# amolrpatil21/PorQua

Hardware: AMD Instinct MI355X
Metric: QPs solved/sec (rebalance dates) at N=1000 assets, 1-8 GPU; x vs host CPU (higher is better)
Workload: dtype f64; 1 GPU; config3: long-only min-variance (P=2*Pearson cov, budget + box [0,1]), daily rebalance; n_assets=1000, window=252, dates_per_gpu=4749, global_batch=4749, parallelism=dates-sharded x1

## Files before the change

include/porqua_hip.h:

```cpp
#ifndef PORQUA_HIP_H
#define PORQUA_HIP_H

#include <stdint.h>

#ifdef __cplusplus
extern "C" {
#endif

#define PQ_VERSION 100

#define PQ_UNSOLVED 0
#define PQ_SOLVED 1
#define PQ_SOLVED_INACCURATE 2
#define PQ_MAX_ITER 3
#define PQ_NEED_REFACTOR 4
#define PQ_PRIMAL_INFEASIBLE (-3)
#define PQ_DUAL_INFEASIBLE (-4)
#define PQ_NON_CONVEX (-5)

#define PQ_OUT_OBJ 0
#define PQ_OUT_PRIM 1
#define PQ_OUT_DUAL 2
#define PQ_OUT_GAP 3
#define PQ_OUT_RHO 4
// ... 155 lines not shown
  double* grho;
  double* M; double* Minv; int32_t k_ld; int64_t M_stride;
  double* aq; int64_t aq_stride;
  double* hinv; int32_t ldh;
  int32_t gmax;
} pq_gcap;
int pq_gcap_assemble(const pq_lowrank* lr, const pq_problem* pb, const pq_gcap* gc, const pq_settings* s,
                     const double* band, int64_t ldo, int32_t r0, const double* pc, int64_t ldpc,
                     const double* cc, void* stream);
int pq_gcap_prepare(const pq_lowrank* lr, const pq_problem* pb, pq_state* st, const pq_gcap* gc,
                    const pq_settings* s, const int32_t* idx, int32_t nidx, const double* band, int64_t ldo,
                    int32_t r0, const double* pc, int64_t ldpc, void* stream);
int pq_admm_lr_gcap(const pq_lowrank* lr, const pq_problem* pb, pq_state* st, const pq_gcap* gc,
                    const pq_settings* s, int32_t iters_this_call, const double* pc, int64_t ldpc, int32_t r0,
                    const double* cc, const int32_t* cg_nzr, const double* cg_nzv, int32_t nzmax, void* stream);
int pq_gcap_form(int32_t gmax, int32_t mg);

int pq_eigcap_form(const pq_lowrank* lr, const pq_problem* pb, const pq_state* st, const pq_settings* s,
                   const int32_t* pdate, const double* V, const double* evals, const double* What,
                   const double* cc, int32_t k_ld, const int32_t* idx, int32_t nidx, double* Minv,
                   int64_t M_stride, double* scratch, void* stream);

int pq_polish_batched(const pq_problem* pb, pq_state* st, const int32_t* idx, int32_t nidx,
                      const pq_settings* s, void* stream);

int pq_polish_lr_batched(const pq_lowrank* lr, const pq_problem* pb, pq_state* st,
                         const int32_t* idx, int32_t nidx, const pq_settings* s, void* stream);

int pq_polish_w_batched(const pq_lowrank* lr, const pq_problem* pb, pq_state* st, const int32_t* idx,
                        int32_t nidx, const pq_settings* s, int32_t ldk, int32_t final_try,
                        const double* band, int64_t ldo, int32_t r0, void* stream);

#define PQ_PG_RECORD 384
#define PQ_PG_PASS_SCRATCH 123537
#define PQ_PG_PENDING 0
#define PQ_PG_DONE 1
#define PQ_PG_FALLBACK 2
#define PQ_PG_SKIP 3
#define PQ_PG_WMB 8
#define PQ_PG_WSCR(k_ld) (2 * PQ_PG_WMB * (int64_t)(k_ld))
typedef struct pq_pg_wide {
  const pq_gcap* gc;
  const double* pc; int64_t ldpc; int32_t r0; const double* cc;
  const int32_t* nzr; const double* nzv; int32_t nzmax;
  double* wscr; int64_t wscr_stride;
  int32_t refine_steps;
} pq_pg_wide;
int pq_polish_grouped_init(const pq_lowrank* lr, const pq_problem* pb, pq_state* st, double* rec,
                           const pq_settings* s, void* stream);
int pq_polish_grouped_round(const pq_lowrank* lr, const pq_problem* pb, pq_state* st, double* rec, int32_t ldk,
                            const int32_t* gdates, int32_t ngroups, const int32_t* urows, const int32_t* ucnt,
                            const int32_t* uoff, int32_t umax, const pq_settings* s, double* pass_scratch,
                            const pq_pg_wide* wide, void* stream);

int pq_simulate_periods(const double* panel, int64_t ldp, int32_t n, const double* W, int64_t ldw,
                        const int32_t* row0, const int32_t* nrows, int32_t nper,
                        const int64_t* ret_off, const int32_t* ret_day, double fc,
                        double days_per_year, double* ret, double* wend, int64_t ldwe,
                        double* turnover, int32_t rescale, void* stream);

int pq_gemv_batched(const double* U, int64_t ldu, int64_t su, int32_t m, int32_t n, int32_t batch,
                    int32_t trans, const double* x, int64_t sx, double* y, int64_t sy, void* stream);

int pq_lad_mv_batched(const double* M, int64_t ldm, int64_t sm, int32_t n, int32_t batch,
                      const double* V, int64_t sv, int32_t k, const double* S, int64_t ss,
                      double* out, int64_t so, void* stream);

int pq_wgram_batched(const double* U, int64_t ldu, int64_t su, int32_t k, int32_t n, int32_t batch,
                     const double* w, int64_t sw, const double* r, int64_t sr, const double* d, int64_t sd,
                     double* M, int32_t k_ld, int64_t sm, void* stream);

int64_t pq_workspace_bytes(int32_t n, int32_t batch, int32_t mg, int32_t path, int32_t tmax, int32_t ldk);


int64_t pq_sym_eig_work_doubles(int32_t ld);
int pq_sym_eig_batched(double* A, int32_t ld, int64_t a_stride, int32_t n, int32_t batch, double* V,
                       int64_t v_stride, double* evals, int64_t e_stride, double* work, int64_t w_stride,
                       int32_t max_sweeps, double tol, void* stream);

int pq_sym_eig_converged(const double* work, int32_t ld, int64_t w_stride, int32_t batch, int32_t max_sweeps,
                         int32_t* conv, void* stream);

int pq_psd_form_batched(const double* V, int64_t v_stride, const double* evals, int64_t e_stride, int32_t ld,
                        int32_t n, int32_t batch, double* out, int64_t o_stride, void* stream);

int pq_tile_gemm_batched(const double* A, int64_t sa, int32_t ta, const double* B, int64_t sb, int32_t tb,
                         double* C, int64_t sc, int32_t ld, int32_t batch, void* stream);

#define PQ_PCT_OK 0
#define PQ_PCT_EMPTY_BUCKET 1
#define PQ_PCT_NAN_SCORE 2
#define PQ_PCT_MAX_N 16384
#define PQ_PCT_MAX_BUCKETS 256
int pq_percentile_batched(const double* scores, int64_t lds, int32_t n, int32_t batch, double sign,
                          int32_t n_percentiles, const int32_t* prev, const int32_t* next,
                          const double* gamma, double* th, int32_t* bucket, int32_t* counts, double* w,
                          int32_t* status, void* stream);

int pq_shrink_stats_band(const double* band, int64_t ldo, int32_t r0, int32_t nrows, int32_t W,
                         const int32_t* rows, int64_t ld_rows, const int32_t* tlen, int32_t tmax,
                         int32_t batch, int32_t n, int32_t centred, int32_t kind, double* stats,
                         void* stream);

#define PQ_RP_OK 0
#define PQ_RP_MAX_SWEEPS 1
#define PQ_RP_BAD_INPUT 2
// ... 63 lines not shown
```

porqua_amd/_lib.py:

```python
from __future__ import annotations

import ctypes
import os

_HERE = os.path.dirname(os.path.abspath(__file__))
LIB_PATH = os.environ.get("PQ_LIB_PATH") or os.path.join(_HERE, "libporqua_hip.so")

c_int32 = ctypes.c_int32
c_int64 = ctypes.c_int64
c_dp = ctypes.c_void_p

PQ_UNSOLVED = 0
PQ_SOLVED = 1
PQ_SOLVED_INACCURATE = 2
PQ_MAX_ITER = 3
PQ_NEED_REFACTOR = 4
PQ_PRIMAL_INFEASIBLE = -3
PQ_DUAL_INFEASIBLE = -4
PQ_NON_CONVEX = -5

PQ_PCT_OK, PQ_PCT_EMPTY_BUCKET, PQ_PCT_NAN_SCORE = range(3)
PQ_PCT_MAX_N = 16384
PQ_PCT_MAX_BUCKETS = 256

# ... 143 lines not shown
    "pq_init_state_lr": ([ctypes.POINTER(PQLowRank), ctypes.POINTER(PQProblem), ctypes.POINTER(PQState), c_dp,
                          c_int32, ctypes.POINTER(PQSettings), c_dp], c_int32),
    "pq_polish_w_batched": ([ctypes.POINTER(PQLowRank), ctypes.POINTER(PQProblem), ctypes.POINTER(PQState),
                             c_dp, c_int32, ctypes.POINTER(PQSettings), c_int32, c_int32, c_dp, c_int64,
                             c_int32, c_dp], c_int32),
    "pq_gram_xy_grouped": ([c_dp, c_int64, c_int32, c_dp, c_dp, c_int32, c_dp, c_int32, c_dp, c_dp, c_dp,
                            c_int64, c_dp, c_dp, c_int64, c_dp], c_int32),
    "pq_gram_xy_batched": ([c_dp, c_int64, c_int32, c_dp, c_dp, c_dp, c_int32, c_int32, c_dp, c_int64,
                            c_dp, c_dp], c_int32),
    "pq_init_state": ([ctypes.POINTER(PQProblem), ctypes.POINTER(PQState), c_dp, c_int32,
                       ctypes.POINTER(PQSettings), c_dp], c_int32),
    "pq_factor_batched": ([ctypes.POINTER(PQProblem), ctypes.POINTER(PQState), c_dp, c_int32,
                           ctypes.POINTER(PQSettings), c_int32, c_dp], c_int32),
    "pq_factor_last_route": ([], c_int32),
    "pq_factor_res_prof": ([c_dp, c_int32], c_int32),
    "pq_factor_large": ([ctypes.POINTER(PQProblem), ctypes.POINTER(PQState), c_dp, c_int32,
                         ctypes.POINTER(PQSettings), c_int32, c_dp, c_int64, c_dp], c_int32),
    "pq_sym_eig_work_doubles": ([c_int32], c_int64),
    "pq_sym_eig_batched": ([c_dp, c_int32, c_int64, c_int32, c_int32, c_dp, c_int64, c_dp, c_int64, c_dp, c_int64,
                            c_int32, ctypes.c_double, c_dp], c_int32),
    "pq_sym_eig_converged": ([c_dp, c_int32, c_int64, c_int32, c_int32, c_dp, c_dp], c_int32),
    "pq_psd_form_batched": ([c_dp, c_int64, c_dp, c_int64, c_int32, c_int32, c_int32, c_dp, c_int64, c_dp], c_int32),
    "pq_tile_gemm_batched": ([c_dp, c_int64, c_int32, c_dp, c_int64, c_int32, c_dp, c_int64, c_int32, c_int32,
                              c_dp], c_int32),
    "pq_admm_batched": ([ctypes.POINTER(PQProblem), ctypes.POINTER(PQState), c_dp, c_int32,
                         ctypes.POINTER(PQSettings), c_int32, c_dp], c_int32),
    "pq_polish_batched": ([ctypes.POINTER(PQProblem), ctypes.POINTER(PQState), c_dp, c_int32,
                           ctypes.POINTER(PQSettings), c_dp], c_int32),
    "pq_admm_lr_grouped": ([ctypes.POINTER(PQLowRank), ctypes.POINTER(PQProblem), ctypes.POINTER(PQState),
                            c_dp, c_int32, c_int64, c_dp, c_int32, c_dp, c_dp, c_dp, c_int32,
                            ctypes.POINTER(PQSettings), c_int32, c_dp, c_int64, c_int32, c_dp, c_dp, c_dp,
                            c_int32, c_dp], c_int32),
    "pq_admm_lr_sweep": ([ctypes.POINTER(PQLowRank), ctypes.POINTER(PQProblem), ctypes.POINTER(PQState),
                          c_dp, c_int32, c_int64, c_dp, c_int32, ctypes.POINTER(PQSettings), c_int32, c_dp,
                          c_int64, c_int32, c_dp, c_int32, c_dp, c_int64, c_dp], c_int32),
    "pq_sweep_scratch_doubles": ([c_int32, c_int32, c_int32], c_int64),
    "pq_polish_lr_batched": ([ctypes.POINTER(PQLowRank), ctypes.POINTER(PQProblem), ctypes.POINTER(PQState),
                              c_dp, c_int32, ctypes.POINTER(PQSettings), c_dp], c_int32),
    "pq_lr_capacitance": ([ctypes.POINTER(PQLowRank), ctypes.POINTER(PQProblem), ctypes.POINTER(PQState),
                           c_dp, c_int32, ctypes.POINTER(PQSettings), c_dp, c_int32, c_int64, c_dp], c_int32),
    "pq_lr_band_gram": ([c_dp, c_int64, c_int32, c_int32, c_int32, c_int32, c_dp, c_int64, c_dp, c_int32, c_int32,
                         c_dp, c_int64, c_dp], c_int32),
    "pq_lr_capacitance_band": ([ctypes.POINTER(PQLowRank), ctypes.POINTER(PQProblem), ctypes.POINTER(PQState),
                                c_dp, c_int32, ctypes.POINTER(PQSettings), c_dp, c_int64, c_int32, c_dp, c_int64,
                                c_dp, c_dp, c_int32, c_int64, c_dp], c_int32),
    "pq_admm_lr_batched": ([ctypes.POINTER(PQLowRank), ctypes.POINTER(PQProblem), ctypes.POINTER(PQState),
                            c_dp, c_int32, c_int64, c_dp, c_int32, ctypes.POINTER(PQSettings), c_int32,
                            c_dp], c_int32),
    "pq_polish_grouped_init": ([ctypes.POINTER(PQLowRank), ctypes.POINTER(PQProblem), ctypes.POINTER(PQState),
                                c_dp, ctypes.POINTER(PQSettings), c_dp], c_int32),
    "pq_polish_grouped_round": ([ctypes.POINTER(PQLowRank), ctypes.POINTER(PQProblem), ctypes.POINTER(PQState),
                                 c_dp, c_int32, c_dp, c_int32, c_dp, c_dp, c_dp, c_int32,
                                 ctypes.POINTER(PQSettings), c_dp, ctypes.POINTER(PQPgWide), c_dp], c_int32),
    "pq_gcap_assemble": ([ctypes.POINTER(PQLowRank), ctypes.POINTER(PQProblem), ctypes.POINTER(PQGcap),
                          ctypes.POINTER(PQSettings), c_dp, c_int64, c_int32, c_dp, c_int64, c_dp, c_dp], c_int32),
    "pq_gcap_prepare": ([ctypes.POINTER(PQLowRank), ctypes.POINTER(PQProblem), ctypes.POINTER(PQState),
                         ctypes.POINTER(PQGcap), ctypes.POINTER(PQSettings), c_dp, c_int32, c_dp, c_int64, c_int32,
                         c_dp, c_int64, c_dp], c_int32),
    "pq_admm_lr_gcap": ([ctypes.POINTER(PQLowRank), ctypes.POINTER(PQProblem), ctypes.POINTER(PQState),
                         ctypes.POINTER(PQGcap), ctypes.POINTER(PQSettings), c_int32, c_dp, c_int64, c_int32, c_dp,
                         c_dp, c_dp, c_int32, c_dp], c_int32),
    "pq_gcap_form": ([c_int32, c_int32], c_int32),
    "pq_eigcap_form": ([ctypes.POINTER(PQLowRank), ctypes.POINTER(PQProblem), ctypes.POINTER(PQState),
                        ctypes.POINTER(PQSettings), c_dp, c_dp, c_dp, c_dp, c_dp, c_int32, c_dp, c_int32, c_dp,
                        c_int64, c_dp, c_dp], c_int32),
    "pq_gemv_batched": ([c_dp, c_int64, c_int64, c_int32, c_int32, c_int32, c_int32, c_dp, c_int64, c_dp,
                         c_int64, c_dp], c_int32),
    "pq_workspace_bytes": ([c_int32, c_int32, c_int32, c_int32, c_int32, c_int32], c_int64),
    "pq_simulate_periods": ([c_dp, c_int64, c_int32, c_dp, c_int64, c_dp, c_dp, c_int32, c_dp, c_dp,
                             ctypes.c_double, ctypes.c_double, c_dp, c_dp, c_int64, c_dp, c_int32, c_dp], c_int32),
    "pq_lad_mv_batched": ([c_dp, c_int64, c_int64, c_int32, c_int32, c_dp, c_int64, c_int32, c_dp, c_int64,
                           c_dp, c_int64, c_dp], c_int32),
    "pq_wgram_batched": ([c_dp, c_int64, c_int64, c_int32, c_int32, c_int32, c_dp, c_int64, c_dp, c_int64,
                          c_dp, c_int64, c_dp, c_int32, c_int64, c_dp], c_int32),
    "pq_percentile_batched": ([c_dp, c_int64, c_int32, c_int32, ctypes.c_double, c_int32, c_dp, c_dp, c_dp,
                               c_dp, c_dp, c_dp, c_dp, c_dp, c_dp], c_int32),
    "pq_shrink_stats_band": ([c_dp, c_int64, c_int32, c_int32, c_int32, c_dp, c_int64, c_dp, c_int32, c_int32,
                              c_int32, c_int32, c_int32, c_dp, c_dp], c_int32),
    "pq_risk_parity_batched": ([ctypes.POINTER(PQLowRank), c_int32, c_int32, c_dp, c_dp, c_dp, c_int64,
                                ctypes.c_double, ctypes.c_double, c_int32, c_dp, c_int64, c_dp, c_dp, c_dp],
                               c_int32),
    "pq_hrp_batched": ([c_dp, c_int64, c_int32, c_int32, c_dp, c_dp, ctypes.c_double, c_dp, c_int64, c_dp, c_int64,
                        c_dp, c_dp, c_dp, c_dp], c_int32),
    "pq_hrp_linkage_batched": ([c_dp, c_int64, c_int32, c_int32, c_dp, c_dp, ctypes.c_double, c_int32, c_dp, c_int64,
                                c_dp, c_int64, c_dp, c_int64, c_dp, c_dp, c_dp, c_dp], c_int32),
    "pq_window_gram_batched": ([c_dp, c_int64, c_int32, c_dp, c_dp, c_int32, c_int32, c_dp, c_int64, c_dp, c_int32,
                                c_int64, c_dp], c_int32),
    "pq_window_project_batched": ([c_dp, c_int64, c_int32, c_dp, c_dp, c_int32, c_int32, c_dp, c_int64, c_dp,
                                   c_int32, c_int64, c_dp, c_dp, c_dp, c_int32, c_dp, c_dp, c_int64, c_dp], c_int32),
    "pq_gerber_cov_batched": ([c_dp, c_int64, c_int32, c_dp, c_dp, c_int32, c_int32, c_dp, c_int64,
                               ctypes.c_double, c_int32, c_int32, c_int32, c_dp, c_dp, c_int64, c_dp, c_int32,
                               c_int64, c_dp, c_dp], c_int32),
    "pq_rank_cov_batched": ([c_dp, c_int64, c_int32, c_dp, c_dp, c_int32, c_int32, c_dp, c_int64, c_int32, c_int32,
                             c_int32, c_dp, c_int64, c_dp, c_int64, c_dp, c_int32, c_int64, c_dp, c_dp], c_int32),
}

_lib = None


def load() -> ctypes.CDLL:
    global _lib
    if _lib is not None:
        return _lib
    if not os.path.exists(LIB_PATH):
        raise PorquaHipError(
            f"{LIB_PATH} not found: build it with `make -C porqua_amd/csrc` "
# ... 19 lines not shown
```

porqua_amd/csrc/polish_g.hip:

```cpp
#include <cstdlib>
#include <mutex>

#include "pg_solve_dev.h"
#include "capi_util.h"

namespace pq {


__global__ __launch_bounds__(PT) void k_pg_init(pq_lowrank lr, pq_problem pb, pq_state st, double* rec,
                                                pq_settings s) {
  __shared__ double red[16];
  const int b = blockIdx.x;
  const int t = threadIdx.x;
  double* R = rec + (int64_t)b * PGR;
  const int st0 = st.status[b];
  if (st0 != PQ_SOLVED && st0 != PQ_MAX_ITER) {
    if (t == 0) R[R_STATE] = PQ_PG_SKIP;
    return;
  }
  const int n = pb.n, ld = pb.ld, mg = pb.mg;
  const double ps = pb.p_scale ? pb.p_scale[b] : 1.0;
  const double pd = pb.p_diag ? pb.p_diag[b] : 0.0;
  const double psw = ps * (lr.w_scale ? lr.w_scale[b] : 1.0);
  const double* q = pb.q + (int64_t)b * pb.q_stride;
// ... 10 lines not shown
  double sc = 0.0;
  for (int i = t; i < n; i += PT) sc = fmax(sc, fmax(fabs(q[i]), fabs(psw * dgb[i] + pd)));
  sc = block_max(sc, red);
  sc = fmax(sc, 1e-300);
  double fix_thr = -INFINITY;
  if (s.polish_fix_rel > 0.0 && has_box && lr.mu) {
    double dm = 0.0;
    for (int i = t; i < n; i += PT)
      if (!isinf(lb[i])) dm = fmax(dm, sx[i] - lb[i]);
    fix_thr = s.polish_fix_rel * block_max(dm, red);
  }
  double nfree = 0.0;
  for (int i = t; i < ld; i += PT) {
    int f = 0;
    if (i < n && has_box) f = start_box(sz[st.mg_pad + i], sy[st.mg_pad + i], sx[i], lb[i], ub[i], fix_thr);
    wk.fl[i] = (i < n) ? f : 1;
    wk.xs[i] = (i < n) ? sx[i] : 0.0;
    nfree += (i < n && f == 0) ? 1.0 : 0.0;
  }
  nfree = block_sum(nfree, red);
  if (t < 64) {
    int a = 0;
    double lam = 0.0;
    if (t < mg) {
      a = start_row(sz[t], sy[t], lg[t], ug[t]);
      lam = sy[t];
    }
    R[R_ACT + t] = a;
    R[R_LAM + t] = lam;
  }
  if (t == 0) {
    R[R_STATE] = PQ_PG_PENDING;
    R[R_ROUNDS] = 0;
    R[R_SC] = sc;
    R[R_K] = nfree;
    R[R_NZB] = 0;
    R[R_W] = 0;
    R[R_FORMED] = 0;
    R[R_REUSE] = 0;
  }
#ifdef PQ_PROFILE
  if (t >= 8 && t < 32) R[t] = 0.0;
#endif
}

__global__ __launch_bounds__(PT) void k_pg_setup(pq_problem pb, pq_state st, double* rec, int kmax, int wide_ok,
                                                 int kbig) {
  __shared__ int wcnt[PW];
  __shared__ int s_al[PG_MGMAX + 1];
  __shared__ double red[16];
  const int b = blockIdx.x;
  double* R = rec + (int64_t)b * PGR;
  if (b == 0 && threadIdx.x == 0) *reinterpret_cast<unsigned long long*>(rec + R_SFLAG) = 0ull;
  if (R[R_STATE] != PQ_PG_PENDING) return;
  const int n = pb.n, ld = pb.ld, mg = pb.mg;
  const int t = threadIdx.x, w = wave_id(), l = lane_id();
  const double* q = pb.q + (int64_t)b * pb.q_stride;
  const double* Cg = pb.Cg ? pb.Cg + (int64_t)b * pb.Cg_stride : nullptr;
  const double* lg = pb.lg ? pb.lg + (int64_t)b * pb.g_stride : nullptr;
  const double* ug = pb.ug ? pb.ug + (int64_t)b * pb.g_stride : nullptr;
  const bool has_box = pb.lb != nullptr;
  const double* lb = has_box ? pb.lb + (int64_t)b * pb.box_stride : nullptr;
  const double* ub = has_box ? pb.ub + (int64_t)b * pb.box_stride : nullptr;
  PGWork wk(st, b, ld);
  const int seg = ((n + PW * 64 - 1) / (PW * 64)) * 64;
  const int lo = w * seg, hi = min(n, lo + seg);
  int c = 0;
  for (int i0 = lo; i0 < hi; i0 += 4 * 64) {
    int fv[4];
#pragma unroll
    for (int u = 0; u < 4; ++u) {
      const int i = i0 + 64 * u + l;
      fv[u] = wk.fl[i < hi ? i : lo];
    }
#pragma unroll
    for (int u = 0; u < 4; ++u) c += __popcll(__ballot(i0 + 64 * u + l < hi && fv[u] == 0));
  }
  if (l == 0) wcnt[w] = c;
  if (t == 0) {
    int a = 0;
    for (int r = 0; r < mg && a <= PG_MGMAX; ++r)
      if (R[R_ACT + r] != 0.0) s_al[a++] = r;
    s_al[PG_MGMAX] = a;
  }
  __syncthreads();
  int base = 0, k = 0;
  for (int ww = 0; ww < PW; ++ww) {
    if (ww < w) base += wcnt[ww];
    k += wcnt[ww];
  }
  const int ma = s_al[PG_MGMAX];
  const int nfx = n - k;
  if (wide_ok && k > kmax && mg <= PG_WG_MAX && ma + nfx <= PG_WMB) {
    if (w == 0) {
      int nb = 0;
      for (int i0 = 0; i0 < n; i0 += 64) {
        const int i = i0 + l;
        const int f = i < n ? wk.fl[i] : 0;
        const unsigned long long m = __ballot(f != 0);
        if (f != 0) {
          const int j = nb + __popcll(m & ((1ull << l) - 1ull));
          R[R_FIX + j] = i;
          R[R_FIXV + j] = f == 1 ? lb[i] : ub[i];
          R[R_FXL + j] = st.y[(int64_t)b * st.m_ld + st.mg_pad + i];
        }
        nb += __popcll(m);
// ... 1223 lines not shown
      __syncthreads();
      if (factor_s()) {
        if (t == 0) R[R_STATE] = PQ_PG_FALLBACK;
        return;
      }
    } else {
      fwd_solve(K, ldk, Dt, nbk, rx, t1, t64, y64p);
    }
    for (int a = w; a < ma; a += PW) {
      double sum = 0.0;
      for (int p = l; p < k; p += 64) sum += U[(int64_t)a * ld + p] * t1[p];
      sum = wave_sum(sum);
      if (l == 0) wl[a] = sum - rl[a];
    }
    __syncthreads();
    if (t == 0) schur_solve(Sm, WMA, ma, wl);
    __syncthreads();
    for (int p = t; p < kp; p += PT) {
      double v = t1[p];
      for (int a = 0; a < ma; ++a) v -= U[(int64_t)a * ld + p] * wl[a];
      t1[p] = v;
    }
    __syncthreads();
    bwd_solve(K, ldk, Dt, nbk, t1, dx, t64, part, y64p);
    for (int p = t; p < k; p += PT) sx[p] += dx[p];
    if (t < ma) lamv[t] += wl[t];
    __syncthreads();
    PG_STAMP(R, 28);
  }
  pg_expand<PT>(t, wk, n, k, sx, ma, s_al, lamv, R);
  PG_STAMP(R, 29);
  if (t == 0) {
    R[30] += 1.0;
    R[31] += (double)k;
  }
}

__global__ __launch_bounds__(PT, 2) void k_pg_big(pq_lowrank lr, pq_problem pb, pq_state st, double* rec,
                                                 pq_settings s, int ldk, int kmin) {
  const int cnt = (int)pg_count(rec, PG_BIGB);
  for (int i = blockIdx.x; i < cnt; i += gridDim.x) {
    pg_big_date(pg_listed(rec, PG_BIGB, i), lr, pb, st, rec, s, ldk, kmin);
    __syncthreads();
  }
}

constexpr int QT = 512;
constexpr int QNW = QT / 64;
constexpr int QG = 16;
constexpr int QU = 320;

constexpr int QS = 4;
constexpr int QCOL = 2048;

struct PassGroup {
  int grp, part, d0, G, U;
};

template <int MODE>
__device__ __forceinline__ bool pass_setup(const PassGroup& pg, const pq_lowrank& lr, const double* rec,
                                           const int32_t* uoff, int* g_on, int* g_T, int* g_off, int* s_any) {
  const int t = threadIdx.x;
  if (t < QG) {
    int on = 0;
    if (t < pg.G) {
      const double* R = rec + (int64_t)(pg.d0 + t) * PGR;
      on = R[R_STATE] == PQ_PG_PENDING && (MODE == 1 || R[R_NZB] != 0.0);
      g_T[t] = lr.tlen[pg.d0 + t];
      g_off[t] = uoff[pg.d0 + t];
    }
    g_on[t] = on;
  }
  __syncthreads();
  if (t == 0) {
    int any = 0;
    for (int g = 0; g < pg.G; ++g) any |= g_on[g];
    *s_any = any;
  }
  __syncthreads();
  return *s_any != 0;
}

__device__ __forceinline__ PassGroup pass_group(const int32_t* gdates, const int32_t* ucnt_all) {
  const int id = xcd_slot(blockIdx.x, gridDim.x);
  PassGroup pg;
  pg.grp = id / QS;
  pg.part = id % QS;
  pg.d0 = gdates[pg.grp];
  pg.G = gdates[pg.grp + 1] - pg.d0;
  pg.U = ucnt_all[pg.grp];
  return pg;
}

constexpr int64_t QSCR = (int64_t)QS * (QU + 4) * QG + QS * QG + QG;

template <int MODE>
__global__ __launch_bounds__(QT) void k_pg_passA(pq_lowrank lr, pq_problem pb, pq_state st, const double* rec,
                                                 const int32_t* gdates, const int32_t* urows_all,
                                                 const int32_t* ucnt_all, const int32_t* uoff, int umax,
                                                 double* scr) {
  __shared__ int s_urow[QU];
  __shared__ int g_on[QG], g_T[QG], g_off[QG];
  __shared__ int s_any;
  __shared__ int s_col[QCOL], s_wcnt[QNW], s_ncol;
  const PassGroup pg = pass_group(gdates, ucnt_all);
  const int U = pg.U, G = pg.G, d0 = pg.d0;
// ... 156 lines not shown
      double a = 0.0;
      for (int q = 0; q < QS; ++q) a += S[(int64_t)q * (QU + 4) * QG + e];
      const bool inw = m < G && g_on[m] && u >= g_off[m] && u < g_off[m] + g_T[m];
      v = inw ? a - g_mux[m] : 0.0;
    }
    WU[e] = v;
  }
  __syncthreads();
  if (pg.part == 0 && t < QG) {
    double a = 0.0;
    for (int u = 0; u < U; ++u) a += WU[u * QG + t];
    scr[pg.grp * QSCR + (int64_t)QS * (QU + 4) * QG + QS * QG + t] = a;
  }
  const int kq = l >> 4, m = l & 15;
  const int Uk = (U + 3) & ~3;
  double* dst = nullptr;
  if (m < G && g_on[m]) {
    PGWork wk(st, d0 + m, ld);
    dst = MODE == 0 ? wk.pxb : wk.g;
  }
  const int nch = (n + 31) / 32;
  const int cper = (nch + QS - 1) / QS;
  const int p_lo = pg.part * cper, p_hi = min(nch, p_lo + cper);
  for (int p = p_lo + w; p < p_hi; p += QNW) {
    const int col = p * 32 + 2 * m;
    const bool cin = col < n;
    f64x4 ce = f64x4{0.0, 0.0, 0.0, 0.0}, co = f64x4{0.0, 0.0, 0.0, 0.0};
    const int colc = cin ? col : 0;
    for (int u0 = 0; u0 < Uk; u0 += 16) {
      double2 a[4];
#pragma unroll
      for (int h = 0; h < 4; ++h) {
        const int u = u0 + 4 * h + kq;
        a[h] = *reinterpret_cast<const double2*>(lr.panel + (int64_t)s_urow[u < U ? u : 0] * lr.ldp + colc);
      }
#pragma unroll
      for (int h = 0; h < 4; ++h) {
        const double bv = WU[(u0 + 4 * h + kq) * QG + m];
        ce = __builtin_amdgcn_mfma_f64_16x16x4f64(a[h].x, bv, ce, 0, 0, 0);
        co = __builtin_amdgcn_mfma_f64_16x16x4f64(a[h].y, bv, co, 0, 0, 0);
      }
    }
    if (dst) {
#pragma unroll
      for (int r = 0; r < 4; ++r) {
        const int i = p * 32 + 2 * (kq + 4 * r);
        if (i < n) dst[i] = ce[r];
        if (i + 1 < n) dst[i + 1] = co[r];
      }
    }
  }
}

constexpr int PPT = 256;
__device__ __forceinline__ double row_dot4(const double* a, const double* b, int n, int hl) {
  double sum = 0.0;
  for (int j0 = hl; j0 < n; j0 += 4 * PPT) {
    double av[4], bv[4];
#pragma unroll
    for (int u = 0; u < 4; ++u) {
      const int j = j0 + u * PPT, jc = j < n ? j : 0;
      av[u] = a[jc];
      bv[u] = b[jc];
    }
#pragma unroll
    for (int u = 0; u < 4; ++u)
      if (j0 + u * PPT < n) sum += av[u] * bv[u];
  }
  return sum;
}
template <int MODE>
__global__ __launch_bounds__(PPT) void k_pg_post(pq_lowrank lr, pq_problem pb, pq_state st, double* rec,
                                                pq_settings s, const int32_t* gdates, int ngroups,
                                                const double* scr) {
  const int b = blockIdx.x;
  double* R = rec + (int64_t)b * PGR;
  if (MODE == 0 && b == 0 && threadIdx.x < PG_NBUCKET)
    reinterpret_cast<unsigned long long*>(rec + R_CNT)[threadIdx.x] = 0ull;
  auto left_for_host = [&]() { *reinterpret_cast<unsigned long long*>(rec + R_SFLAG) = 1ull; };
  if (MODE == 1 && R[R_STATE] != PQ_PG_PENDING && threadIdx.x == 0) {
    const int stt = st.status[b];
    if (R[R_STATE] == PQ_PG_FALLBACK || stt == PQ_NEED_REFACTOR || stt == PQ_SOLVED_INACCURATE || stt == PQ_UNSOLVED)
      left_for_host();
  }
  if (!(R[R_STATE] == PQ_PG_PENDING && (MODE == 1 || R[R_NZB] != 0.0))) return;
  int lo = 0, hi = ngroups;
  while (hi - lo > 1) {
    const int mid = (lo + hi) >> 1;
    if (gdates[mid] <= b) lo = mid; else hi = mid;
  }
  const int grp = lo, hg = b - gdates[grp];
  __shared__ double red[16];
  const int hl = threadIdx.x;
  const int n = pb.n, ld = pb.ld, mg = pb.mg;
  PGWork wk(st, b, ld);
  const double* mu = lr.mu ? lr.mu + (int64_t)b * lr.mu_stride : nullptr;
  const double su = scr[(int64_t)grp * QSCR + (int64_t)QS * (QU + 4) * QG + QS * QG + hg];
  const double wsc = lr.w_scale ? lr.w_scale[b] : 1.0;
  if (MODE == 0) {
    for (int i = hl; i < n; i += PPT) wk.pxb[i] = wsc * (wk.pxb[i] - (mu ? mu[i] * su : 0.0));
    return;
  }
  const double ps = pb.p_scale ? pb.p_scale[b] : 1.0;
  const double pd = pb.p_diag ? pb.p_diag[b] : 0.0;
  const double* q = pb.q + (int64_t)b * pb.q_stride;
  const double* Cg = pb.Cg ? pb.Cg + (int64_t)b * pb.Cg_stride : nullptr;
  const double* lg = pb.lg ? pb.lg + (int64_t)b * pb.g_stride : nullptr;
  const double* ug = pb.ug ? pb.ug + (int64_t)b * pb.g_stride : nullptr;
  const bool has_box = pb.lb != nullptr;
  const double* lb = has_box ? pb.lb + (int64_t)b * pb.box_stride : nullptr;
  const double* ub = has_box ? pb.ub + (int64_t)b * pb.box_stride : nullptr;
  const double sc = R[R_SC];
  const double dtol = s.dual_tol * sc;
  const double ptol = 1e-12;
  const double soft = s.polish_release_rel > 0.0 ? s.polish_release_rel * sc : 0.0;
  const bool vtx = R[R_K] == 0.0 && R[R_MA] == 1.0;
  const int r0 = vtx ? (int)R[R_AL] : -1;
  double lam0 = 0.0;
  if (vtx) {
    const double* c0 = Cg + (int64_t)r0 * ld;
    double lo = -INFINITY, hi = INFINITY;
    for (int i = hl; i < n; i += PPT) {
      const int f = wk.fl[i];
      const double c = c0[i];
      if (f == 0 || c == 0.0 || (has_box && lb[i] == ub[i])) continue;
      const double pxi = ps * (wsc * (wk.g[i] - (mu ? mu[i] * su : 0.0))) + pd * wk.xs[i];
      const double bnd = -(pxi + q[i]) / c;
      if ((f == 1) == (c > 0.0)) lo = fmax(lo, bnd);
      else hi = fmin(hi, bnd);
    }
    lo = block_max(lo, red);
    hi = -block_max(-hi, red);
    lam0 = (isfinite(lo) && isfinite(hi)) ? 0.5 * (lo + hi) : (isfinite(lo) ? lo : (isfinite(hi) ? hi : 0.0));
  }
  auto lamof = [&](int r) -> double { return r == r0 ? lam0 : R[R_LAM + r]; };
  int bad = 0;
  const double lam_r0 = mg > 0 ? lamof(0) : 0.0;
  for (int i0 = hl; i0 < n; i0 += 4 * PPT) {
    double xv[4], gv[4], mv4[4], qv[4], c0[4], lbv[4], ubv[4];
    int fv[4];
#pragma unroll
    for (int j = 0; j < 4; ++j) {
      const int i = i0 + j * PPT, ic = i < n ? i : 0;
      xv[j] = wk.xs[ic];
      gv[j] = wk.g[ic];
      mv4[j] = mu ? mu[ic] : 0.0;
      qv[j] = q[ic];
      c0[j] = mg > 0 ? Cg[ic] : 0.0;
      fv[j] = wk.fl[ic];
      lbv[j] = has_box ? lb[ic] : 0.0;
      ubv[j] = has_box ? ub[ic] : 0.0;
    }
#pragma unroll
// ... 185 lines not shown

static int pg_big() {
  static const int v = [] {
    const char* e = getenv("PQ_PG_BIG");
    return e ? atoi(e) : 1;
  }();
  return v;
}

static int solve_rt() {
  static const int v = [] {
    const char* e = getenv("PQ_PG_RT");
    return e ? atoi(e) : 4;
  }();
  return v;
}

static int solve_waves(int bucket) {
  static const int forced = [] {
    const char* e = getenv("PQ_PG_SOLVE_NW");
    const int v = e ? atoi(e) : 0;
    return v == 1 || v == 2 || v == 4 ? v : 0;
  }();
  static const int def[5] = {2, 2, 4, 4, 4};
  return forced ? forced : def[bucket];
}

template <int KS>
static void launch_solve_ks(int nw, int B, hipStream_t str, const pq_problem* pb, pq_state* st, double* rec,
                            const pq_settings* s, int ldk, int klo) {
  const int inner = s->polish_inner > 0 ? s->polish_inner : 0;
  if (nw == 1)
    hipLaunchKernelGGL((k_pg_solve<KS, 1>), dim3(resident_grid((const void*)k_pg_solve<KS, 1>, 64, B)), dim3(64), 0,
                       str, *pb, *st, rec, *s, ldk, klo, inner);
  else if (nw == 2)
    hipLaunchKernelGGL((k_pg_solve<KS, 2>), dim3(resident_grid((const void*)k_pg_solve<KS, 2>, 128, B)), dim3(128),
                       0, str, *pb, *st, rec, *s, ldk, klo, inner);
  else
    hipLaunchKernelGGL((k_pg_solve<KS, 4>), dim3(resident_grid((const void*)k_pg_solve<KS, 4>, 256, B)), dim3(256),
                       0, str, *pb, *st, rec, *s, ldk, klo, inner);
}
static void launch_solve(int bucket, int nw, int B, hipStream_t str, const pq_problem* pb, pq_state* st,
                         double* rec, const pq_settings* s, int ldk, int klo) {
  switch (bucket) {
    case 0: launch_solve_ks<48>(nw, B, str, pb, st, rec, s, ldk, klo); break;
    case 1: launch_solve_ks<64>(nw, B, str, pb, st, rec, s, ldk, klo); break;
    case 2: launch_solve_ks<80>(nw, B, str, pb, st, rec, s, ldk, klo); break;
    case 3: launch_solve_ks<96>(nw, B, str, pb, st, rec, s, ldk, klo); break;
    default: launch_solve_ks<128>(nw, B, str, pb, st, rec, s, ldk, klo); break;
  }
}
}

extern "C" int pq_polish_grouped_round(const pq_lowrank* lr, const pq_problem* pb, pq_state* st, double* rec,
                                       int32_t ldk, const int32_t* gdates, int32_t ngroups, const int32_t* urows,
                                       const int32_t* ucnt, const int32_t* uoff, int32_t umax, const pq_settings* s,
                                       double* pass_scratch, const pq_pg_wide* wide, void* stream) {
  PQ_CHECK_ARG(lr && pb && st && s && rec && pass_scratch, "pq_polish_grouped_round: null argument");
  static_assert(pq::QSCR == pq::GB_OFF && pq::GB_END == PQ_PG_PASS_SCRATCH, "PQ_PG_PASS_SCRATCH out of date");
  PQ_CHECK_ARG(gdates && urows && ucnt && uoff && umax > 0 && umax <= pq::QU,
               "pq_polish_grouped_round: group plan missing (umax <= %d)", pq::QU);
  PQ_CHECK_ARG(pb->n % 2 == 0 && lr->ldp % 2 == 0, "pq_polish_grouped_round: needs even n and panel stride");
  PQ_CHECK_ARG(pb->mg >= 0 && pb->mg <= pq::PG_MGMAX, "pq_polish_grouped_round: mg <= %d", pq::PG_MGMAX);
  PQ_CHECK_ARG(st->K && ldk >= 64 && st->K_stride >= (int64_t)ldk * ldk,
               "pq_polish_grouped_round: K scratch (ldk x ldk per problem) too small");
  if (pb->batch <= 0 || ngroups <= 0) return 0;
  hipStream_t str = (hipStream_t)stream;
  const int B = pb->batch;
  const int kmax = ldk < pq::PG_KMAX ? ldk : pq::PG_KMAX;
  const int kbig = (pq::pg_big() && ldk > kmax) ? (ldk < pq::PG_KBIG ? ldk : pq::PG_KBIG) : kmax;
  hipLaunchKernelGGL(pq::k_pg_setup, dim3(B), dim3(pq::PT), 0, str, *pb, *st, rec, kmax, wide ? 1 : 0, kbig);
  const dim3 gsplit(ngroups * pq::QS);
  hipLaunchKernelGGL(pq::k_pg_passA<0>, gsplit, dim3(pq::QT), 0, str, *lr, *pb, *st, rec, gdates, urows, ucnt, uoff,
                     umax, pass_scratch);
  hipLaunchKernelGGL(pq::k_pg_passB<0>, gsplit, dim3(pq::QT), 0, str, *lr, *pb, *st, rec, gdates, urows, ucnt, uoff,
                     umax, pass_scratch);
  hipLaunchKernelGGL(pq::k_pg_post<0>, dim3(B), dim3(pq::PPT), 0, str, *lr, *pb, *st, rec, *s, gdates, ngroups,
                     pass_scratch);
  if (pq::group_form_min() > 0)
    hipLaunchKernelGGL(pq::k_pg_form_grp, dim3(ngroups), dim3(pq::FT), 0, str, *lr, *pb, *st, rec, gdates, urows,
                       ucnt, umax, pass_scratch, pq::group_form_min());
  hipLaunchKernelGGL(pq::k_pg_form<pq::PG_KMAX>, dim3(B), dim3(pq::FT), 0, str, *lr, *pb, *st, rec, ldk, gdates, ngroups, urows,
                     ucnt, uoff, umax, pass_scratch);
  pq::PgSide* side = pq::pg_side();
  int used = 0;
  if (side && hipEventRecord(side->fork, str) != hipSuccess) side = nullptr;
  auto on = [&](int i) -> hipStream_t {
    if (!side || hipStreamWaitEvent(side->s[i], side->fork, 0) != hipSuccess) return str;
    used |= 1 << i;
    return side->s[i];
  };
  if (kbig > kmax) {
    static_assert(pq::PG_KBIG == 256, "k_pg_form<PG_KBIG> tiling");
    const hipStream_t sb = on(6);
    if (pq::group_form_big_min() > 0 && lr->mu == nullptr)
      hipLaunchKernelGGL(pq::k_pg_form_grp_big, dim3(ngroups * pq::GBS), dim3(pq::FT), 0, sb, *lr, *pb, *st, rec,
                         gdates, urows, ucnt, umax, pass_scratch, pq::group_form_big_min());
    hipLaunchKernelGGL(pq::k_pg_form<pq::PG_KBIG>, dim3(pq::resident_grid((const void*)pq::k_pg_form<pq::PG_KBIG>,
                                                                          pq::FT, B)),
                       dim3(pq::FT), 0, sb, *lr, *pb, *st, rec, ldk, gdates, ngroups, urows, ucnt, uoff, umax,
                       pass_scratch);
    hipLaunchKernelGGL(pq::k_pg_big, dim3(pq::resident_grid((const void*)pq::k_pg_big, pq::PT, B)), dim3(pq::PT), 0,
                       sb, *lr, *pb, *st, rec, *s, ldk, kmax);
  }
  const int nrt = pq::solve_rt() <= 0 ? 0 : (pq::solve_rt() >= 4 ? 4 : 3);
  for (int i = 4; i >= nrt; --i) {
    static const int KSB[5] = {48, 64, 80, 96, 128};
    if (i >= 2 && kmax <= KSB[i - 1]) continue;
    pq::launch_solve(i, pq::solve_waves(i), B, on(i), pb, st, rec, s, ldk, i ? KSB[i - 1] : 0);
  }
  if (nrt > 0 && pq_pg_solve_rt_launch(nrt + 2, B, on(1), pb, st, rec, s, ldk)) return -1;
  if (wide && pq_pg_wide_launch(lr, pb, st, rec, s, wide, on(5))) return -1;
  for (int i = 0; side && i < pq::PgSide::NS; ++i)
    if ((used & (1 << i)) && (hipEventRecord(side->join[i], side->s[i]) != hipSuccess ||
                              hipStreamWaitEvent(str, side->join[i], 0) != hipSuccess)) {
      pq::set_error("pq_polish_grouped_round: joining the solve streams failed");
      return -2;
    }
  hipLaunchKernelGGL(pq::k_pg_passA<1>, gsplit, dim3(pq::QT), 0, str, *lr, *pb, *st, rec, gdates, urows, ucnt, uoff,
                     umax, pass_scratch);
  hipLaunchKernelGGL(pq::k_pg_passB<1>, gsplit, dim3(pq::QT), 0, str, *lr, *pb, *st, rec, gdates, urows, ucnt, uoff,
                     umax, pass_scratch);
  hipLaunchKernelGGL(pq::k_pg_post<1>, dim3(B), dim3(pq::PPT), 0, str, *lr, *pb, *st, rec, *s, gdates, ngroups,
                     pass_scratch);
  PQ_CHECK_LAUNCH("pq_polish_grouped_round");
  return 0;
}

int pq::resident_grid(const void* kernel, int block, int B) {
  struct Entry { const void* k; int dev, n; };
  static Entry cache[64];
  static int used = 0;
  static std::mutex mu;
  int dev = 0;
  if (hipGetDevice(&dev) != hipSuccess) return B;
  std::lock_guard<std::mutex> lock(mu);
  for (int i = 0; i < used; ++i)
    if (cache[i].k == kernel && cache[i].dev == dev) return cache[i].n < B ? cache[i].n : B;
  int per = 0, cus = 0;
  if (hipOccupancyMaxActiveBlocksPerMultiprocessor(&per, kernel, block, 0) != hipSuccess ||
      hipDeviceGetAttribute(&cus, hipDeviceAttributeMultiprocessorCount, dev) != hipSuccess || per <= 0 || cus <= 0) {
    (void)hipGetLastError();
    return B;
  }
  const int n = per * cus;
  if (used < 64) cache[used++] = Entry{kernel, dev, n};
  return n < B ? n : B;
}
```

Measured before the change: 779,100 QPs/s.

## Fuse polish passA/passB into one kernel and fold pass-0 post-scaling

```diff
diff --git a/include/porqua_hip.h b/include/porqua_hip.h
--- a/include/porqua_hip.h
+++ b/include/porqua_hip.h
@@ -231,6 +231,7 @@
                             const int32_t* gdates, int32_t ngroups, const int32_t* urows, const int32_t* ucnt,
                             const int32_t* uoff, int32_t umax, const pq_settings* s, double* pass_scratch,
                             const pq_pg_wide* wide, void* stream);
+int pq_pg_pass_form(int32_t n);
 
 int pq_simulate_periods(const double* panel, int64_t ldp, int32_t n, const double* W, int64_t ldw,
                         const int32_t* row0, const int32_t* nrows, int32_t nper,
diff --git a/porqua_amd/_lib.py b/porqua_amd/_lib.py
--- a/porqua_amd/_lib.py
+++ b/porqua_amd/_lib.py
@@ -219,6 +219,7 @@
     "pq_polish_grouped_round": ([ctypes.POINTER(PQLowRank), ctypes.POINTER(PQProblem), ctypes.POINTER(PQState),
                                  c_dp, c_int32, c_dp, c_int32, c_dp, c_dp, c_dp, c_int32,
                                  ctypes.POINTER(PQSettings), c_dp, ctypes.POINTER(PQPgWide), c_dp], c_int32),
+    "pq_pg_pass_form": ([c_int32], c_int32),
     "pq_gcap_assemble": ([ctypes.POINTER(PQLowRank), ctypes.POINTER(PQProblem), ctypes.POINTER(PQGcap),
                           ctypes.POINTER(PQSettings), c_dp, c_int64, c_int32, c_dp, c_int64, c_dp, c_dp], c_int32),
     "pq_gcap_prepare": ([ctypes.POINTER(PQLowRank), ctypes.POINTER(PQProblem), ctypes.POINTER(PQState),
diff --git a/porqua_amd/csrc/polish_g.hip b/porqua_amd/csrc/polish_g.hip
--- a/porqua_amd/csrc/polish_g.hip
+++ b/porqua_amd/csrc/polish_g.hip
@@ -86,6 +86,8 @@
   const int b = blockIdx.x;
   double* R = rec + (int64_t)b * PGR;
   if (b == 0 && threadIdx.x == 0) *reinterpret_cast<unsigned long long*>(rec + R_SFLAG) = 0ull;
+  if (b == 0 && threadIdx.x < PG_NBUCKET)
+    reinterpret_cast<unsigned long long*>(rec + R_CNT)[threadIdx.x] = 0ull;
   if (R[R_STATE] != PQ_PG_PENDING) return;
   const int n = pb.n, ld = pb.ld, mg = pb.mg;
   const int t = threadIdx.x, w = wave_id(), l = lane_id();
@@ -1415,6 +1417,8 @@
 
 constexpr int QS = 4;
 constexpr int QCOL = 2048;
+constexpr int QFUSE = 512;
+static_assert(QFUSE <= QCOL, "the fused pass has the compacted form only");
 
 struct PassGroup {
   int grp, part, d0, G, U;
@@ -1677,6 +1681,230 @@
   }
 }
 
+#ifndef PQ_PG_PASS0_FOLD
+#define PQ_PG_PASS0_FOLD 1
+#endif
+#ifndef PQ_PG_PASS1_FUSED
+#define PQ_PG_PASS1_FUSED 0
+#endif
+
+__device__ __forceinline__ double pass0_entry(double raw, const double* mu, int i, double su, double wsc) {
+  return wsc * (raw - (mu ? mu[i] * su : 0.0));
+}
+
+template <int MODE>
+__global__ __launch_bounds__(QT, 6) void k_pg_pass(pq_lowrank lr, pq_problem pb, pq_state st, const double* rec,
+                                                const int32_t* gdates, const int32_t* urows_all,
+                                                const int32_t* ucnt_all, const int32_t* uoff, int umax,
+                                                double* scr) {
+  constexpr bool FOLD = MODE == 0 && PQ_PG_PASS0_FOLD != 0;
+  __shared__ __attribute__((aligned(16))) double WU[(QU + 16) * QG];
+  __shared__ int s_urow[QU];
+  __shared__ int g_on[QG], g_T[QG], g_off[QG];
+  __shared__ double g_mux[QG], g_su[QG];
+  __shared__ int s_any;
+  constexpr int NZW = QS * QCOL / 64;
+  static_assert(QS * QCOL <= 65536 && QT == 512, "s_col entries and the bit words of a 512-column step");
+  __shared__ unsigned long long s_nz[NZW];
+  __shared__ int s_pre[NZW + 1];
+  __shared__ unsigned short s_col[QCOL];
+  const PassGroup pg = pass_group(gdates, ucnt_all);
+  const int U = pg.U, G = pg.G, d0 = pg.d0;
+  const int t = threadIdx.x, w = wave_id(), l = lane_id();
+  const int n = pb.n, ld = pb.ld;
+  for (int u = t; u < QU; u += QT) s_urow[u] = u < U ? urows_all[(int64_t)pg.grp * umax + u] : 0;
+  if (!pass_setup<MODE>(pg, lr, rec, uoff, g_on, g_T, g_off, &s_any)) return;
+  const int per = ((n + QS - 1) / QS + 7) & ~7;
+  for (int cb = 0; cb < n; cb += QT) {
+    const int i = cb + t;
+    const int ic = i < n ? i : 0;
+    double v[QG];
+#pragma unroll
+    for (int g = 0; g < QG; ++g) {
+      PGWork wg(st, d0 + (g < G ? g : 0), ld);
+      v[g] = (MODE == 0 ? wg.xb : wg.xs)[ic];
+    }
+    bool nz = false;
+#pragma unroll
+    for (int g = 0; g < QG; ++g) nz |= g < G && g_on[g] && v[g] != 0.0;
+    const unsigned long long bal = __ballot(nz && i < n);
+    if (l == 0) s_nz[(cb >> 6) + w] = bal;
+  }
+  {
+    const int hg = t >> 5, hl = t & 31;
+    const bool act = hg < G && g_on[hg];
+    PGWork wk(st, d0 + (act ? hg : 0), ld);
+    const double* v = MODE == 0 ? wk.xb : wk.xs;
+    const double* mu = (act && lr.mu) ? lr.mu + (int64_t)(d0 + hg) * lr.mu_stride : nullptr;
+    double tot = 0.0;
+    for (int q = 0; q < QS; ++q) {
+      const int k_lo = q * per, k_hi = min(n, k_lo + per);
+      double a = 0.0;
+      if (mu)
+        for (int i0 = k_lo + hl; i0 < k_hi; i0 += 8 * 32) {
+          double mv[8], vv[8];
+#pragma unroll
+          for (int e = 0; e < 8; ++e) {
+            const int i = i0 + 32 * e, ic = i < k_hi ? i : k_lo;
+            mv[e] = mu[ic];
+            vv[e] = v[ic];
+          }
+#pragma unroll
+          for (int e = 0; e < 8; ++e)
+            if (i0 + 32 * e < k_hi) a = fma(mv[e], vv[e], a);
+        }
+      a = lanes_sum<32>(a);
+      tot += a;
+    }
+    if (hl == 0) g_mux[hg] = tot;
+  }
+  __syncthreads();
+  const int nzw = (n + 63) >> 6;
+  if (t <= nzw) {
+    int a = 0;
+    for (int ww = 0; ww < t; ++ww) a += __popcll(s_nz[ww]);
+    s_pre[t] = a;
+  }
+  __syncthreads();
+  auto below = [&](int i) -> int {
+    const int r = i & 63;
+    return s_pre[i >> 6] + (r ? __popcll(s_nz[i >> 6] & ((1ull << r) - 1ull)) : 0);
+  };
+  auto list = [&](int lo, int hi) {
+    const int base = below(lo);
+    for (int i = lo + t; i < hi; i += QT)
+      if ((s_nz[i >> 6] >> (i & 63)) & 1ull) s_col[below(i) - base] = (unsigned short)i;
+  };
+  const bool whole = s_pre[nzw] <= QCOL;
+  if (whole) list(0, n);
+  const int ntile = (U + 15) >> 4;
+  const int kq = l >> 4, m = l & 15;
+  const double* Vp = nullptr;
+  if (m < G && g_on[m]) {
+    PGWork wk(st, d0 + m, ld);
+    Vp = MODE == 0 ? wk.xb : wk.xs;
+  }
+  const double* Vq = Vp ? Vp : lr.panel;
+  const double* arow[3];
+#pragma unroll
+  for (int j = 0; j < 3; ++j) {
+    const int u = (w + QNW * j) * 16 + m;
+    arow[j] = lr.panel + (int64_t)s_urow[u < QU ? u : 0] * lr.ldp;
+  }
+  double* const Wc = WU + (w * 16 + kq) * QG + m;
+  constexpr int WJ = QNW * 16 * QG, WR = 4 * QG;
+  const bool t2 = (w + 2 * QNW) * 16 < QU + 16;
+#pragma unroll
+  for (int j = 0; j < 3; ++j)
+    if (j < 2 || t2) {
+#pragma unroll
+      for (int r = 0; r < 4; ++r) Wc[j * WJ + r * WR] = 0.0;
+    }
+  if (whole) __syncthreads();
+  for (int q = 0; q < QS; ++q) {
+    const int k_lo = min(n, q * per), k_hi = min(n, k_lo + per);
+    if (!whole) {
+      __syncthreads();
+      list(k_lo, k_hi);
+      __syncthreads();
+    }
+    const int cbase = whole ? below(k_lo) : 0;
+    const int ncol = below(k_hi) - below(k_lo);
+    f64x4 c[3];
+#pragma unroll
+    for (int j = 0; j < 3; ++j) c[j] = f64x4{0.0, 0.0, 0.0, 0.0};
+    for (int k0 = 0; k0 < ncol; k0 += 16) {
+      double av[4][3], bv[4];
+#pragma unroll
+      for (int h = 0; h < 4; ++h) {
+        const int kk = k0 + 4 * h + kq;
+        const bool kin = kk < ncol;
+        const int col = s_col[cbase + (kin ? kk : 0)];
+        bv[h] = Vq[col] * ((Vp && kin) ? 1.0 : 0.0);
+#pragma unroll
+        for (int j = 0; j < 3; ++j) av[h][j] = arow[j][col];
+      }
+#pragma unroll
+      for (int h = 0; h < 4; ++h)
+#pragma unroll
+        for (int j = 0; j < 3; ++j) c[j] = __builtin_amdgcn_mfma_f64_16x16x4f64(av[h][j], bv[h], c[j], 0, 0, 0);
+    }
+#pragma unroll
+    for (int j = 0; j < 3; ++j)
+      if (j < 2 || t2) {
+#pragma unroll
+        for (int r = 0; r < 4; ++r) Wc[j * WJ + r * WR] += c[j][r];
+      }
+  }
+  {
+    const bool on_m = m < G && g_on[m];
+    const int u_lo = g_off[m], u_hi = on_m ? min(u_lo + g_T[m], ntile * 16) : u_lo;
+    const double mux = g_mux[m];
+#pragma unroll
+    for (int j = 0; j < 3; ++j)
+      if (j < 2 || t2) {
+#pragma unroll
+        for (int r = 0; r < 4; ++r) {
+          const int u = (w + QNW * j) * 16 + kq + 4 * r;
+          const double a = Wc[j * WJ + r * WR];
+          Wc[j * WJ + r * WR] = (u >= u_lo && u < u_hi) ? a - mux : 0.0;
+        }
+      }
+  }
+  __syncthreads();
+  if ((FOLD || pg.part == 0) && t < QG) {
+    double a = 0.0;
+    for (int u = 0; u < U; ++u) a += WU[u * QG + t];
+    if (FOLD) g_su[t] = a;
+    if (pg.part == 0) scr[pg.grp * QSCR + (int64_t)QS * (QU + 4) * QG + QS * QG + t] = a;
+  }
+  if (FOLD) __syncthreads();
+  const int Uk = (U + 3) & ~3;
+  double* dst = nullptr;
+  const double* mu_m = nullptr;
+  double su_m = 0.0, wsc_m = 1.0;
+  if (m < G && g_on[m]) {
+    PGWork wk(st, d0 + m, ld);
+    dst = MODE == 0 ? wk.pxb : wk.g;
+    if (FOLD) {
+      mu_m = lr.mu ? lr.mu + (int64_t)(d0 + m) * lr.mu_stride : nullptr;
+      su_m = g_su[m];
+      wsc_m = lr.w_scale ? lr.w_scale[d0 + m] : 1.0;
+    }
+  }
+  const int nch = (n + 31) / 32;
+  const int cper = (nch + QS - 1) / QS;
+  const int p_lo = pg.part * cper, p_hi = min(nch, p_lo + cper);
+  for (int p = p_lo + w; p < p_hi; p += QNW) {
+    const int col = p * 32 + 2 * m;
+    const bool cin = col < n;
+    f64x4 ce = f64x4{0.0, 0.0, 0.0, 0.0}, co = f64x4{0.0, 0.0, 0.0, 0.0};
+    const int colc = cin ? col : 0;
+    for (int u0 = 0; u0 < Uk; u0 += 16) {
+      double2 a[4];
+#pragma unroll
+      for (int h = 0; h < 4; ++h) {
+        const int u = u0 + 4 * h + kq;
+        a[h] = *reinterpret_cast<const double2*>(lr.panel + (int64_t)s_urow[u < U ? u : 0] * lr.ldp + colc);
+      }
+#pragma unroll
+      for (int h = 0; h < 4; ++h) {
+        const double bv = WU[(u0 + 4 * h + kq) * QG + m];
+        ce = __builtin_amdgcn_mfma_f64_16x16x4f64(a[h].x, bv, ce, 0, 0, 0);
+        co = __builtin_amdgcn_mfma_f64_16x16x4f64(a[h].y, bv, co, 0, 0, 0);
+      }
+    }
+    if (dst) {
+#pragma unroll
+      for (int r = 0; r < 4; ++r) {
+        const int i = p * 32 + 2 * (kq + 4 * r);
+        if (i < n) dst[i] = FOLD ? pass0_entry(ce[r], mu_m, i, su_m, wsc_m) : ce[r];
+        if (i + 1 < n) dst[i + 1] = FOLD ? pass0_entry(co[r], mu_m, i + 1, su_m, wsc_m) : co[r];
+      }
+    }
+  }
+}
+
 constexpr int PPT = 256;
 __device__ __forceinline__ double row_dot4(const double* a, const double* b, int n, int hl) {
   double sum = 0.0;
@@ -1700,8 +1928,6 @@
                                                 const double* scr) {
   const int b = blockIdx.x;
   double* R = rec + (int64_t)b * PGR;
-  if (MODE == 0 && b == 0 && threadIdx.x < PG_NBUCKET)
-    reinterpret_cast<unsigned long long*>(rec + R_CNT)[threadIdx.x] = 0ull;
   auto left_for_host = [&]() { *reinterpret_cast<unsigned long long*>(rec + R_SFLAG) = 1ull; };
   if (MODE == 1 && R[R_STATE] != PQ_PG_PENDING && threadIdx.x == 0) {
     const int stt = st.status[b];
@@ -1723,7 +1949,7 @@
   const double su = scr[(int64_t)grp * QSCR + (int64_t)QS * (QU + 4) * QG + QS * QG + hg];
   const double wsc = lr.w_scale ? lr.w_scale[b] : 1.0;
   if (MODE == 0) {
-    for (int i = hl; i < n; i += PPT) wk.pxb[i] = wsc * (wk.pxb[i] - (mu ? mu[i] * su : 0.0));
+    for (int i = hl; i < n; i += PPT) wk.pxb[i] = pass0_entry(wk.pxb[i], mu, i, su, wsc);
     return;
   }
   const double ps = pb.p_scale ? pb.p_scale[b] : 1.0;
@@ -2015,6 +2241,13 @@
 }
 }
 
+extern "C" int pq_pg_pass_form(int32_t n) {
+  const int per = ((n + pq::QS - 1) / pq::QS + 7) & ~7;
+  if (n <= 0 || per > pq::QFUSE) return 0;
+  const char* e = getenv("PQ_PG_PASS_FUSED");
+  return (e && atoi(e) == 0) ? 0 : 1;
+}
+
 extern "C" int pq_polish_grouped_round(const pq_lowrank* lr, const pq_problem* pb, pq_state* st, double* rec,
                                        int32_t ldk, const int32_t* gdates, int32_t ngroups, const int32_t* urows,
                                        const int32_t* ucnt, const int32_t* uoff, int32_t umax, const pq_settings* s,
@@ -2034,12 +2267,19 @@
   const int kbig = (pq::pg_big() && ldk > kmax) ? (ldk < pq::PG_KBIG ? ldk : pq::PG_KBIG) : kmax;
   hipLaunchKernelGGL(pq::k_pg_setup, dim3(B), dim3(pq::PT), 0, str, *pb, *st, rec, kmax, wide ? 1 : 0, kbig);
   const dim3 gsplit(ngroups * pq::QS);
-  hipLaunchKernelGGL(pq::k_pg_passA<0>, gsplit, dim3(pq::QT), 0, str, *lr, *pb, *st, rec, gdates, urows, ucnt, uoff,
-                     umax, pass_scratch);
-  hipLaunchKernelGGL(pq::k_pg_passB<0>, gsplit, dim3(pq::QT), 0, str, *lr, *pb, *st, rec, gdates, urows, ucnt, uoff,
-                     umax, pass_scratch);
-  hipLaunchKernelGGL(pq::k_pg_post<0>, dim3(B), dim3(pq::PPT), 0, str, *lr, *pb, *st, rec, *s, gdates, ngroups,
-                     pass_scratch);
+  const int fused = pq_pg_pass_form(pb->n);
+  if (fused) {
+    hipLaunchKernelGGL(pq::k_pg_pass<0>, gsplit, dim3(pq::QT), 0, str, *lr, *pb, *st, rec, gdates, urows, ucnt, uoff,
+                       umax, pass_scratch);
+  } else {
+    hipLaunchKernelGGL(pq::k_pg_passA<0>, gsplit, dim3(pq::QT), 0, str, *lr, *pb, *st, rec, gdates, urows, ucnt,
+                       uoff, umax, pass_scratch);
+    hipLaunchKernelGGL(pq::k_pg_passB<0>, gsplit, dim3(pq::QT), 0, str, *lr, *pb, *st, rec, gdates, urows, ucnt,
+                       uoff, umax, pass_scratch);
+  }
+  if (!fused || !PQ_PG_PASS0_FOLD)
+    hipLaunchKernelGGL(pq::k_pg_post<0>, dim3(B), dim3(pq::PPT), 0, str, *lr, *pb, *st, rec, *s, gdates, ngroups,
+                       pass_scratch);
   if (pq::group_form_min() > 0)
     hipLaunchKernelGGL(pq::k_pg_form_grp, dim3(ngroups), dim3(pq::FT), 0, str, *lr, *pb, *st, rec, gdates, urows,
                        ucnt, umax, pass_scratch, pq::group_form_min());
@@ -2080,10 +2320,18 @@
       pq::set_error("pq_polish_grouped_round: joining the solve streams failed");
       return -2;
     }
-  hipLaunchKernelGGL(pq::k_pg_passA<1>, gsplit, dim3(pq::QT), 0, str, *lr, *pb, *st, rec, gdates, urows, ucnt, uoff,
-                     umax, pass_scratch);
-  hipLaunchKernelGGL(pq::k_pg_passB<1>, gsplit, dim3(pq::QT), 0, str, *lr, *pb, *st, rec, gdates, urows, ucnt, uoff,
-                     umax, pass_scratch);
+#if PQ_PG_PASS1_FUSED
+  if (fused) {
+    hipLaunchKernelGGL(pq::k_pg_pass<1>, gsplit, dim3(pq::QT), 0, str, *lr, *pb, *st, rec, gdates, urows, ucnt, uoff,
+                       umax, pass_scratch);
+  } else
+#endif
+  {
+    hipLaunchKernelGGL(pq::k_pg_passA<1>, gsplit, dim3(pq::QT), 0, str, *lr, *pb, *st, rec, gdates, urows, ucnt,
+                       uoff, umax, pass_scratch);
+    hipLaunchKernelGGL(pq::k_pg_passB<1>, gsplit, dim3(pq::QT), 0, str, *lr, *pb, *st, rec, gdates, urows, ucnt,
+                       uoff, umax, pass_scratch);
+  }
   hipLaunchKernelGGL(pq::k_pg_post<1>, dim3(B), dim3(pq::PPT), 0, str, *lr, *pb, *st, rec, *s, gdates, ngroups,
                      pass_scratch);
   PQ_CHECK_LAUNCH("pq_polish_grouped_round");
```

Result: no change. 775,000 QPs/s (-0.5%).
